# Alvin-Zeng/DRN

Hardware: AMD Instinct MI355X
Metric: clips/sec fwd+bwd (BxT=256x4096 C3D feats) (higher is better)
Workload: dtype bf16; 1 GPU; Charades-STA-shaped C3D features, T=256, D=4096, batch 32/GPU, stage-1 losses; step = fwd+bwd+grad all-reduce+clip(0.5)+Adam; global_batch=32, T=256, D=4096, parallelism=dp1

## Files before the change

drn_amd/csrc/bn.hip:

```cpp
#include "vec.h"
#include "bn_merge.h"
#include "../../include/drn_hip.h"

struct BnFinGroup {
  const float* stats;
  int tiles, M;
  float* scale_shift;
  float* save;
  const float* gamma;
  const float* beta;
  const float* conv_bias;
  float* running_mean;
  float* running_var;
  float momentum, eps;
};
struct BnFinParams {
  int ngroups;
  BnFinGroup g[DRN_MAX_GROUPS];
};

__global__ __launch_bounds__(256 * DRN_MAX_GROUPS) void bn_finalize_kernel(const BnFinParams P, int C) {
  __shared__ double sh[DRN_MAX_GROUPS][16][17];
  __shared__ float s_mean[DRN_MAX_GROUPS][16], s_unb[DRN_MAX_GROUPS][16];
  const int g = threadIdx.x >> 8, t = threadIdx.x & 255;
// ... 388 lines not shown
          const float y = fmaf(u1[k], sc1[k], sh1[k]);
          u1[k] = relu ? fmaxf(y, 0.f) : y;
        }
        if (raw2) {
          float u2[N];
          V16<T>::cvt(ur2[u], u2);
#pragma unroll
          for (int k = 0; k < N; ++k) {
            const float y = fmaf(u2[k], sc2[k], sh2[k]);
            u1[k] += DT<T>::round(relu ? fmaxf(y, 0.f) : y);
          }
        }
#pragma unroll
        for (int k = 0; k < N; ++k) x[k] += DT<T>::round(u1[k]);
      } else if (up) {
        float uu[N];
        V16<T>::cvt(ur[u], uu);
#pragma unroll
        for (int k = 0; k < N; ++k) x[k] += uu[k];
      }
      if (m < row1) {
        V16<T>::store(out + (long)m * ld_out + c0, x);
        if (gated) {
          const float* gp = gate + (long)sq[u] * ldg + c0;
#pragma unroll
          for (int k = 0; k < N; ++k) x[k] *= gp[k];
          V16<T>::store(gated + (long)m * ld_gated + c0, x);
        }
      }
    }
  }
}

extern "C" int drn_bn_train_apply(const DrnBnTrainDesc* d, int n, int C, int relu, int dtype, void* stream) {
  drn_clear_status();
  const char* who = "drn_bn_train_apply";
  DRN_CHECK_ARG(d && n >= 1 && n <= DRN_MAX_GROUPS && C > 0 && C % 64 == 0, "%s: bad args (C must be a multiple of 64)", who);
  DRN_CHECK_ARG(dtype == DRN_F32 || dtype == DRN_BF16, "%s: bad dtype %d", who, dtype);
  const int vn = dtype == DRN_BF16 ? 8 : 4;
  const int RP = 256 / (64 / vn);
  BnTrainParams P;
  memset(&P, 0, sizeof(P));
  P.n = n; P.C = C; P.relu = relu; P.nupd = C / 64;
  long m_all = 0;
  for (int i = 0; i < n; ++i) m_all += d[i].M;
  const long wg4 = ((m_all + 4 * RP - 1) / (4 * RP)) * (C / 64);
  const int rows_wg = 4 * RP * (int)(wg4 > 4096 ? (wg4 + 4095) / 4096 : 1);
  int blocks = P.nupd;
  for (int i = 0; i < n; ++i) {
    const DrnBnTrainDesc& s = d[i];
    DRN_CHECK_ARG(s.raw && s.out && s.stats && s.scale_shift && s.save && s.gamma && s.beta && s.M > 0 && s.L > 0 && s.M % s.L == 0 &&
                  s.tiles == (s.M + 127) / 128, "%s: bad level %d", who, i);
    DRN_CHECK_ARG(!s.up || (s.L % 2 == 0), "%s: upsample-add needs an even sequence length", who);
    DRN_CHECK_ARG((s.gate != nullptr) == (s.gated != nullptr), "%s: gate and gated must come together", who);
    DRN_CHECK_ARG(s.ld_raw % vn == 0 && s.ld_out % vn == 0 && (!s.up || s.ld_up % vn == 0) && (!s.gated || (s.ld_gated % vn == 0 && s.ldg % 4 == 0)),
                  "%s: ld must be 16-byte multiples", who);
    BnTrainLv& G = P.lv[i];
    G.raw = s.raw; G.out = s.out; G.up = s.up; G.gated = s.gated; G.gate = s.gate;
    G.stats = s.stats; G.ss = s.scale_shift; G.save = s.save; G.gamma = s.gamma; G.beta = s.beta; G.conv_bias = s.conv_bias;
    G.running_mean = s.running_mean; G.running_var = s.running_var; G.momentum = s.momentum; G.eps = s.eps;
    G.ld_raw = s.ld_raw; G.ld_out = s.ld_out; G.ld_up = s.ld_up; G.ld_gated = s.ld_gated; G.ldg = s.ldg; G.M = s.M; G.L = s.L;
    G.tiles = s.tiles; G.blk0 = blocks; G.rows_wg = rows_wg;
    blocks += cdiv(s.M, rows_wg) * (C / 64);
    G.chain_next = -1;
    for (int j = 0; j < n && s.up; ++j)
      if (j != i && d[j].out == s.up) {
        DRN_CHECK_ARG(d[j].L * 2 == s.L && d[j].M * 2 == s.M,
                      "%s: level %d adds the output of level %d of the same launch, whose geometry (M=%d L=%d) is not half of its own "
                      "(M=%d L=%d): launch the levels in order", who, i, j, d[j].M, d[j].L, s.M, s.L);
        G.chain_next = j;
        G.up = nullptr;
      }
  }
  for (int i = 0; i < n; ++i) {
    int depth = 1;
    for (int h = P.lv[i].chain_next; h >= 0 && depth <= n; h = P.lv[h].chain_next) ++depth;
    DRN_CHECK_ARG(depth <= 3, "%s: an upsample chain of more than three levels inside one launch (launch the levels in order)", who);
    DRN_CHECK_ARG(P.lv[i].chain_next < 0 || P.lv[i].L % 4 == 0 || P.lv[P.lv[i].chain_next].chain_next < 0,
                  "%s: a three-level chain needs sequence lengths that are multiples of 4", who);
  }
  P.total_blocks = blocks;
  if (dtype == DRN_BF16) bn_train_apply_kernel<bf16_t><<<blocks, 256, 0, (hipStream_t)stream>>>(P);
  else bn_train_apply_kernel<float><<<blocks, 256, 0, (hipStream_t)stream>>>(P);
  return drn_launch_status(who);
}

struct BnBwdLv {
  const void* dout;
  const void* raw;
  void* draw;
  const float* ss;
  const float* save;
  const float* gamma;
  float* dgamma;
  float* dbeta;
  float* partial;
  float* coef;
  int ld_dout, ld_raw, ld_draw, M, accumulate, nblk, yblk0, ablk0;
};
struct BnBwdParams {
  BnBwdLv lv[DRN_MAX_GROUPS];
  int n, C, relu, total_yblk, total_ablk;
};

template <typename T>
__global__ __launch_bounds__(256) void bn_bwd_reduce_kernel(const BnBwdParams P) {
  constexpr int N = V16<T>::N;
  __shared__ float red[2][4][64 * N + 1];
  int li = 0;
#pragma unroll
  for (int i = 1; i < DRN_MAX_GROUPS; ++i)
    if (i < P.n && (int)blockIdx.y >= P.lv[i].yblk0) li = i;
  const BnBwdLv& G = P.lv[li];
  const int C = P.C, relu = P.relu, M = G.M;
// ... 898 lines not shown
```

drn_amd/csrc/bn_merge.h:

```cpp
#pragma once
#include "common.h"

enum { BN_ST_PLAIN = 0, BN_ST_TAGGED = 2 };
struct BnTagged {
  unsigned want;
  int* timeouts;
};
__device__ __forceinline__ unsigned long long bn_tag_pack(float v, unsigned tag) {
  return ((unsigned long long)tag << 32) | (unsigned long long)__float_as_uint(v);
}
__device__ __forceinline__ unsigned long long bn_ld_pair(const unsigned long long* p) {
  return __hip_atomic_load(p, __ATOMIC_RELAXED, __HIP_MEMORY_SCOPE_AGENT);
}
__device__ __forceinline__ bool bn_wait_expired(const long long t0, int* timeouts) {
  __builtin_amdgcn_s_sleep(32);
  if (wall_clock64() - t0 <= 200000000LL) return false;
  __hip_atomic_fetch_add(timeouts, 1, __ATOMIC_RELAXED, __HIP_MEMORY_SCOPE_AGENT);
  return true;
}

__device__ __forceinline__ void bn_wait_slabs(const void* st_, const int slabs, const int C, const int c_first, const BnTagged tg) {
  const unsigned long long* p = (const unsigned long long*)st_ + c_first;
  const int lane = threadIdx.x & 63;
  const long long t0 = wall_clock64();
  for (int s0 = 0; s0 < slabs; s0 += 64) {
    const int s = s0 + lane;
    bool ready = s >= slabs;
    for (;;) {
      if (!ready) ready = (unsigned)(bn_ld_pair(p + ((long)s * 2 + 1) * C) >> 32) == tg.want;
      if (__builtin_amdgcn_ballot_w64(!ready) == 0) break;
      __builtin_amdgcn_s_sleep(12);
      if (wall_clock64() - t0 > 200000000LL) {
        if (!ready) __hip_atomic_fetch_add(tg.timeouts, 1, __ATOMIC_RELAXED, __HIP_MEMORY_SCOPE_AGENT);
        break;
      }
    }
  }
}

template <int CB, int MODE, int TB = 8>
__device__ __forceinline__ void bn_merge_cols(const void* __restrict__ st_, const int tiles, const int Mrows, const int C,
                                              const int cbase, double (*shd)[CB], double& mean_out, double& var_out,
                                              const BnTagged tg = BnTagged{0u, nullptr}) {
#pragma clang fp contract(off)
  constexpr int KMAX = 16;
  const int ci = threadIdx.x % CB, j = threadIdx.x / CB;
  const float* __restrict__ p = (const float*)st_ + cbase;
  const unsigned long long* __restrict__ pt = (const unsigned long long*)st_ + cbase;
  auto at = [&](int k, int which) -> unsigned { return (unsigned)(k * 2 + which) * (unsigned)C + (unsigned)ci; };
  auto ld = [&](int k, int which) -> float {
    if constexpr (MODE == BN_ST_TAGGED) return __uint_as_float((unsigned)bn_ld_pair(pt + at(k, which)));
    else return p[at(k, which)];
  };
  const bool cached = tiles <= 4 * KMAX;
  float c0[KMAX], c1[KMAX];
  double s = 0.0;
  if (cached) {
    if constexpr (MODE == BN_ST_TAGGED) {
      const long long t0 = wall_clock64();
#pragma unroll
      for (int hb = 0; hb < KMAX / TB; ++hb) {
        if (hb > 0 && tiles <= 4 * TB * hb) {
#pragma unroll
          for (int i = hb * TB; i < KMAX; ++i) c0[i] = c1[i] = 0.f;
          break;
        }
        for (;;) {
          bool ok = true;
#pragma unroll
          for (int i = hb * TB; i < (hb + 1) * TB; ++i) {
            const int k = min(j + 4 * i, tiles - 1);
            const unsigned long long v0 = bn_ld_pair(pt + at(k, 0)), v1 = bn_ld_pair(pt + at(k, 1));
            ok &= (unsigned)(v0 >> 32) == tg.want && (unsigned)(v1 >> 32) == tg.want;
            c0[i] = __uint_as_float((unsigned)v0);
            c1[i] = __uint_as_float((unsigned)v1);
          }
          if (ok || bn_wait_expired(t0, tg.timeouts)) break;
        }
      }
// ... 71 lines not shown
```

drn_amd/csrc/gemm_nt.hip:

```cpp
#include "gemm_nt_kernel.h"

bool drn_nt_w4_eligible(const DrnGemmDesc* d, int ngroups, int dtype);
int drn_nt_w4_launch(const GemmParams& P, int total, hipStream_t stream);
bool drn_nt_w4c_eligible(const DrnGemmDesc* d, int ngroups, int dtype);
int drn_nt_w4c_launch(const GemmParams& P, int total, hipStream_t stream, int ksplit, bool eval = false);
bool drn_nt_w4h_eligible(const DrnGemmDesc* d, int ngroups, int dtype, bool* conv_out);
int drn_nt_w4h_launch(const GemmParams& P, int total, bool conv, hipStream_t stream, int ksplit, bool eval = false);

static int nt_kind(const DrnGemmDesc* d, int ngroups, int dtype, int tile, int ksplit, bool planes256) {
  if (tile == 256 && ksplit == 1 && drn_tuning(DRN_TUNE_NT_W4) > 0 && drn_nt_w4_eligible(d, ngroups, dtype)) return DRN_NT_KIND_W4;
  if (tile == 256 && (planes256 || (ksplit == 1 && drn_tuning(DRN_TUNE_NT_W4C) > 0)) && drn_nt_w4c_eligible(d, ngroups, dtype))
    return DRN_NT_KIND_W4C;
  return tile == 256 ? DRN_NT_KIND_TILE256 : DRN_NT_KIND_TILE128;
}

static int launch_nt(const DrnGemmDesc* d, int ngroups, int dtype, hipStream_t stream, int ksplit_arg = 1, float* ws = nullptr,
                     int* counters = nullptr, bool planes256 = false, bool plan_only = false, const DrnBnApplyDesc* ev = nullptr,
                     int ev_relu = 0) {
  const int ksplit = ksplit_arg & 0xffff;
  const int xchg = ksplit_arg & (DRN_XCHG_CONFIRM | DRN_XCHG_NONE);
  DRN_CHECK_ARG(ngroups >= 1 && ngroups <= DRN_MAX_GROUPS, "drn_gemm_nt: ngroups=%d out of range", ngroups);
  DRN_CHECK_ARG(dtype == DRN_F32 || dtype == DRN_BF16, "drn_gemm_nt: bad dtype %d", dtype);
  const int ch = dtype == DRN_BF16 ? 8 : 4;
  long big_tiles = 0;
  bool fast = true;
  for (int g = 0; g < ngroups; ++g) {
    const DrnGemmDesc& s = d[g];
    DRN_CHECK_ARG(s.A && s.B && s.C, "drn_gemm_nt: null operand in group %d", g);
    DRN_CHECK_ARG(s.M > 0 && s.N > 0 && s.Cin > 0 && s.taps >= 1 && s.stride >= 1, "drn_gemm_nt: bad dims in group %d", g);
    DRN_CHECK_ARG(s.Cin % ch == 0 && s.lda % ch == 0 && s.ldb % ch == 0,
                  "drn_gemm_nt: Cin/lda/ldb must be multiples of %d elements (16 bytes); got Cin=%d lda=%d ldb=%d", ch,
                  s.Cin, s.lda, s.ldb);
    DRN_CHECK_ARG(((uintptr_t)s.A & 15) == 0 && ((uintptr_t)s.B & 15) == 0, "drn_gemm_nt: A/B must be 16-byte aligned");
    DRN_CHECK_ARG(s.Lout > 0 && s.Lsrc > 0 && s.M % s.Lout == 0, "drn_gemm_nt: M=%d not a multiple of Lout=%d", s.M, s.Lout);
    big_tiles += (long)cdiv(s.M, 256) * cdiv(s.N, 256);
    if (s.Cin % (8 * ch) != 0 || (s.mode == 1 && s.stride > 2)) fast = false;
  }
  const int big_min = drn_tuning(DRN_TUNE_EXP0) > 0 ? drn_tuning(DRN_TUNE_EXP0) : 200;
  int tile = big_tiles >= big_min ? 256 : 128;
  GemmParams P;
  memset(&P, 0, sizeof(P));
  P.ngroups = ngroups;
  P.ksplit = ksplit | (ksplit > 1 && counters ? (xchg & DRN_XCHG_NONE ? 0 : xchg & DRN_XCHG_CONFIRM ? DRN_XCHG_CONFIRM : DRN_XCHG_READBACK) : 0);
  P.ws = ws;
  P.counters = counters;
  P.xcd_swizzle = 3;
  if (drn_tuning(DRN_TUNE_EXP0 + 3) > 0) P.xcd_swizzle = drn_tuning(DRN_TUNE_EXP0 + 3) - 1;
  if (ksplit > 1) tile = planes256 ? 256 : 128;
  bool w4h = false, w4h_conv = false;
  if (tile == 128 && !planes256 && drn_tuning(DRN_TUNE_NT_W4H) > 0 && drn_nt_w4h_eligible(d, ngroups, dtype, &w4h_conv)) {
    long th = 0;
    int min_ksteps = 1 << 30;
    for (int g = 0; g < ngroups; ++g) {
      th += (long)(d[g].M / 256) * (d[g].N / 128);
      const int ksteps = d[g].taps * d[g].Cin / 64, per = cdiv(ksteps, ksplit);
      min_ksteps = min(min_ksteps, ksteps - (cdiv(ksteps, per) - 1) * per);
      if (cdiv(ksteps, per) != ksplit) min_ksteps = 0;
    }
    w4h = ksplit == 1 ? th >= drn_tuning(DRN_TUNE_NT_W4H)
                      : (ngroups == 1 && th * ksplit >= drn_tuning(DRN_TUNE_NT_W4H) && min_ksteps >= 2 && th <= DRN_QD_COUNTERS && ws && counters);
  }
  const int tile_m = w4h ? 256 : tile, tile_n = w4h ? 128 : tile;
  int total = 0;
  for (int g = 0; g < ngroups; ++g) {
    const DrnGemmDesc& s = d[g];
    GemmProb& p = P.p[g];
    p.A = s.A; p.B = s.B; p.C = s.C; p.C2 = s.C2; p.bias = s.bias; p.gate = s.gate; p.stats = s.stats;
    p.M = s.M; p.N = s.N; p.K = s.taps * s.Cin; p.Cin = s.Cin; p.taps = s.taps; p.stride = s.stride; p.pad = s.pad;
    p.mode = s.mode; p.Lout = s.Lout; p.Lsrc = s.Lsrc; p.lda = s.lda; p.ldb = s.ldb; p.ldc = s.ldc; p.ldg = s.ldg; p.ldc2 = s.ldc2;
    p.accumulate = s.accumulate;
    p.out_f32 = s.out_f32;
    p.sumsq = s.sumsq;
    if (ev) { p.ev_ss = ev[g].scale_shift; p.ev_relu = ev_relu ? 1 : 0; }
    p.gb_act = s.gb_act; p.gb_dct = s.gb_dct; p.gb_dgate = s.gb_dgate; p.gb_dsum = s.gb_dsum; p.gb_ld_act = s.gb_ld_act; p.gb_ldt = s.gb_ldt;
    p.tiles_n = cdiv(s.N, tile_n);
    p.tile_start = total;
    total += cdiv(s.M, tile_m) * p.tiles_n;
  }
  int max_ksteps = 0;
  for (int g = 0; g < ngroups; ++g) max_ksteps = max(max_ksteps, cdiv(cdiv(d[g].taps * d[g].Cin, 8 * ch), ksplit));
  const bool deep8 = tile == 128 &&
                     ((drn_tuning(DRN_TUNE_NT_DEEP) > 0 && (long)total * ksplit <= drn_tuning(DRN_TUNE_NT_DEEP)) ||
                      (drn_tuning(DRN_TUNE_NT_DEEP2) > 0 && (long)total * ksplit <= drn_tuning(DRN_TUNE_NT_DEEP2) &&
                       max_ksteps <= drn_tuning(DRN_TUNE_NT_DEEP_KS)));
  static bool attr_set = false;
  if (!attr_set) {
#define NT_ATTR(TT, SS, ...) \
    (void)hipFuncSetAttribute((const void*)conv_gemm_nt_kernel<TT, SS, true, __VA_ARGS__>, hipFuncAttributeMaxDynamicSharedMemorySize, 163840); \
    (void)hipFuncSetAttribute((const void*)conv_gemm_nt_kernel<TT, SS, false, __VA_ARGS__>, hipFuncAttributeMaxDynamicSharedMemorySize, 163840)
    NT_ATTR(float, 2, 2, 4, 8, 4); NT_ATTR(bf16_t, 2, 2, 4, 8, 4);
    NT_ATTR(float, 2, 2, 4, 4, 2); NT_ATTR(bf16_t, 2, 2, 4, 4, 2);
    NT_ATTR(float, 4, 2, 4, 4, 2); NT_ATTR(bf16_t, 4, 2, 4, 4, 2);
#undef NT_ATTR
#define NT_ATTR(TT, SS, ...) \
    (void)hipFuncSetAttribute((const void*)conv_gemm_nt_eval_kernel<TT, SS, true, __VA_ARGS__>, hipFuncAttributeMaxDynamicSharedMemorySize, 163840); \
    (void)hipFuncSetAttribute((const void*)conv_gemm_nt_eval_kernel<TT, SS, false, __VA_ARGS__>, hipFuncAttributeMaxDynamicSharedMemorySize, 163840)
    NT_ATTR(float, 2, 2, 4, 8, 4); NT_ATTR(bf16_t, 2, 2, 4, 8, 4);
    NT_ATTR(float, 2, 2, 4, 4, 2); NT_ATTR(bf16_t, 2, 2, 4, 4, 2);
    NT_ATTR(float, 4, 2, 4, 4, 2); NT_ATTR(bf16_t, 4, 2, 4, 4, 2);
#undef NT_ATTR
    attr_set = true;
  }
#define NT_LAUNCH(TT, SS, THREADS, LDS, ...) do { \
    P.nblocks = total; \
    if (ev && fast) conv_gemm_nt_eval_kernel<TT, SS, true, __VA_ARGS__><<<dim3(total, ksplit), THREADS, LDS, stream>>>(P); \
    else if (ev) conv_gemm_nt_eval_kernel<TT, SS, false, __VA_ARGS__><<<dim3(total, ksplit), THREADS, LDS, stream>>>(P); \
    else if (fast) conv_gemm_nt_kernel<TT, SS, true, __VA_ARGS__><<<dim3(total, ksplit), THREADS, LDS, stream>>>(P); \
    else conv_gemm_nt_kernel<TT, SS, false, __VA_ARGS__><<<dim3(total, ksplit), THREADS, LDS, stream>>>(P); } while (0)
  const int kind = w4h ? DRN_NT_KIND_W4H : nt_kind(d, ngroups, dtype, tile, ksplit, planes256);
  if (ev && kind == DRN_NT_KIND_W4) {
    drn_set_error("drn_conv_bn_eval: gemm_nt_w4_kernel (large plain products) has no BatchNorm epilogue");
    return DRN_ERR_UNSUPPORTED;
  }
  if (plan_only) return kind;
  if (kind == DRN_NT_KIND_W4H) {
    P.nblocks = total;
    return drn_nt_w4h_launch(P, total, w4h_conv, stream, ksplit, ev != nullptr);
  }
  for (int g = 0; g < ngroups; ++g)
    DRN_CHECK_ARG(!d[g].sumsq || (kind == DRN_NT_KIND_W4 && d[g].out_f32 && !d[g].bias && !d[g].accumulate && ngroups == 1),
                  "drn_gemm_nt: DrnGemmDesc::sumsq needs a single fp32-output launch on gemm_nt_w4_kernel without bias / accumulate "
                  "(ask drn_gemm_nt_plan first)");
  for (int g = 0; g < ngroups; ++g) {
    const DrnGemmDesc& s = d[g];
    if (!s.gb_act) continue;
    DRN_CHECK_ARG(kind == DRN_NT_KIND_W4C && ngroups == 1 && ksplit == 1 && s.mode == 1 && s.gate && s.gb_dct && s.gb_dgate && s.gb_dsum &&
                      !s.bias && !s.C2 && !s.stats && !s.accumulate && (s.Lout == 32 || s.Lout == 64 || s.Lout == 128 || s.Lout == 256) &&
                      s.gb_ld_act % 8 == 0 && s.gb_ldt % 8 == 0 && !((uintptr_t)s.gb_act & 15) && !((uintptr_t)s.gb_dct & 15) && s.ldg >= s.N,
                  "drn_gemm_nt: DrnGemmDesc::gb_* needs a single bf16 data-gradient launch on gemm_nt_w4c_kernel (ask drn_gemm_nt_plan "
                  "first) with gate and all three outputs set, clips of 32 / 64 / 128 / 256 rows, no bias / C2 / stats / accumulate");
  }
  if (kind == DRN_NT_KIND_W4) {
    P.nblocks = total;
    return drn_nt_w4_launch(P, total, stream);
  }
  if (kind == DRN_NT_KIND_W4C) {
    P.nblocks = total;
    return drn_nt_w4c_launch(P, total, stream, ksplit, ev != nullptr);
  }
  if (planes256) {
    drn_set_error("drn_gemm_nt_splitk256: the problem is not one gemm_nt_w4c_kernel runs (bf16, k = 3 / stride 1 / pad 1, M and N multiples of 256, Cin of 64)");
    return DRN_ERR_UNSUPPORTED;
// ... 207 lines not shown
```

drn_amd/csrc/gemm_nt_kernel.h:

```cpp
#pragma once
#include <type_traits>
#include "common.h"
#include "bn_merge.h"
#include "../../include/drn_hip.h"



struct GemmProb {
  const void* A;
  const void* B;
  void* C;
  void* C2;
  union {
    const float* bias;
    const float* ev_ss;
  };
  const float* gate;
  float* stats;
  int M, N, K;
  int Cin, taps, stride, pad, mode;
  int Lout, Lsrc;
  int lda, ldb, ldc, ldg, ldc2;
  union {
    int accumulate;
// ... 395 lines not shown
      const int mrow0 = m0 + wr * (MI * 16) + ch * 32;
#pragma unroll
      for (int mi2 = 0; mi2 < 2; ++mi2)
#pragma unroll
        for (int r = 0; r < 4; ++r)
#pragma unroll
          for (int ni = 0; ni < NI; ++ni)
            *((float*)(wbuf + (mi2 * 16 + (l >> 4) * 4 + r) * PITCHF) + ni * 16 + (l & 15)) = acc[ch * 2 + mi2][ni][r];
      wave_lds_sync();
#pragma unroll
      for (int it = 0; it < 32 / RPIF; ++it) {
        const int rl = it * RPIF + l / LPRF, cv = l % LPRF;
        const int m = mrow0 + rl, n = n0 + wc * (NI * 16) + cv * 4;
        if (m < M && n < N) {
          f32x4 v = *(const f32x4*)(wbuf + rl * PITCHF + cv * 16);
          float* g = Cf + ((long)m * pr.ldc + n);
          if (pr.bias)
#pragma unroll
            for (int k = 0; k < 4; ++k) v[k] += n + k < N ? pr.bias[n + k] : 0.f;
          if (vec4 && n + 4 <= N && !pr.accumulate) {
            *(f32x4*)g = v;
          } else {
#pragma unroll
            for (int k = 0; k < 4; ++k)
              if (n + k < N) g[k] = pr.accumulate ? g[k] + v[k] : v[k];
          }
        }
      }
      wave_lds_sync();
    }
    return;
  }
  auto bn_stats = [&](float* shs) { nt_bn_stats<WM, WN, MI, NI, BN_ST_PLAIN>(acc, shs, pr.stats, M, N, m0, n0, tm); };

  T* __restrict__ Cg = (T*)pr.C;
  T* __restrict__ C2g = (T*)pr.C2;
  constexpr int VEC = 16 / (int)sizeof(T);
  const bool vec_ok = (pr.ldc % VEC == 0) && (((uintptr_t)Cg & 15) == 0) &&
                      (!C2g || ((pr.ldc2 % VEC == 0) && (((uintptr_t)C2g & 15) == 0)));
  const bool stats_first = !vec_ok;
  if (!EVAL && stats_first && pr.stats) {
    bn_stats((float*)smem);
    __syncthreads();
  }
  if (vec_ok) {
    constexpr int WCOLS = NI * 16;
    constexpr int PITCH = WCOLS * (int)sizeof(T) + 16;
    constexpr int LPR = WCOLS * (int)sizeof(T) / 16;
    constexpr int RPI = 64 / LPR;
    char* wbuf = smem + w * (32 * PITCH);
    float bias_v[NI], scale_v[NI];
#pragma unroll
    for (int ni = 0; ni < NI; ++ni) {
      const int n = n0 + wc * (NI * 16) + ni * 16 + (l & 15);
      if constexpr (EVAL) {
        scale_v[ni] = n < N ? pr.ev_ss[n] : 0.f;
        bias_v[ni] = n < N ? pr.ev_ss[N + n] : 0.f;
      } else {
        bias_v[ni] = (pr.bias && n < N) ? pr.bias[n] : 0.f;
      }
    }
    (void)scale_v;
    const int npass = C2g ? 2 : 1;
#pragma unroll
    for (int ch = 0; ch < MI / 2; ++ch) {
      const int mrow0 = m0 + wr * (MI * 16) + ch * 32;
// ... 743 lines not shown
```

drn_amd/functional.py:

```python
import contextlib
import weakref

import torch

from . import ops
from ._lib import DrnError

class WeightCopies(object):

    _live = []

    def __init__(self):
        self.pack, self.pstack, self.stack, self.shape_stack = {}, {}, {}, {}
        self.epoch = 0
        self.gen = 0
        WeightCopies._live.append(weakref.ref(self))

    def bump_gen(self):
        self.gen += 1

    def bump_epoch(self):
        self.epoch += 1

    def adopt(self, module):
# ... 668 lines not shown
        keep = (draws, xs)
        dWj = _alias(dW)
        _defer(lambda: (keep, ops.gemm_wgrad(wdescs, dWj, Cout, Cin, taps=k, stride=meta.stride, pad=pad, w_layout=1, dtype=code)), dWj)
        dxs = [None] * nl
        if any(ctx.needs_input_grad[7 + l] for l in range(nl)):
            wd = packed(ctx.weight_obj, (1, 2, 0), code)
            tail = meta.tail if (meta.tail is not None and nl == 1 and k in (1, 3) and meta.tail.usable(Cin, Cout, dt)) else None
            ncols = Cin - tail.P if tail is not None else Cin
            descs = []
            for l in range(nl):
                B, L, Lo, M, ld = geo[l]
                dx = torch.empty((B, L, Cin), dtype=dt, device=dev)
                descs.append(ops.gemm_desc(draws[l], wd, dx, B * L, ncols, Cout, taps=k, stride=meta.stride, pad=pad, mode=1,
                                           Lout=L, Lsrc=Lo, ldc=Cin))
                dxs[l] = dx
            gctx = tail.gate_ctx if tail is not None else None
            if (gctx is not None and k == 3 and meta.stride == 1 and gctx[2:] == (geo[0][0], geo[0][1], ncols)
                    and ops.gemm_nt_plan(descs, code) == ops.NT_KIND_W4C):
                Z, gate0, B, T, D = gctx
                dZT = torch.empty((D, B * T), dtype=dt, device=dev)
                dgate0 = torch.empty((B, D), dtype=torch.float32, device=dev)
                dsum0 = torch.empty((B, D), dtype=torch.float32, device=dev)
                descs = [ops.gemm_desc(draws[0], wd, dxs[0], B * T, ncols, Cout, taps=k, stride=1, pad=pad, mode=1, Lout=T, Lsrc=T, ldc=Cin,
                                       gate=gate0, ldg=gate0.stride(0),
                                       gate_bwd=dict(act=Z, ld_act=D, dct=dZT, ldt=B * T, dgate=dgate0, dsum=dsum0))]
                tail.gate_out = (dZT, dgate0, dsum0)
            ops.gemm_nt(descs, code)
            if tail is not None:
                B, L, Lo, M, ld = geo[0]
                tail.backward(draws[0], wd, B, L, Lo, Cout, Cin, k, meta.stride, pad, code)
        return (None, dW, None, dgamma, dbeta, dgate, dup) + tuple(dxs)


def conv_block(xs, conv, bn, training, dtype, gate=None, up=None, relu=True, tail=None):
    meta = ConvMeta(conv.stride[0], bn, training, dtype, relu, tail=tail)
    res = _ConvBlockFn.apply(meta, conv.weight, conv.bias, bn.weight, bn.bias, gate, up, *xs)
    if gate is not None:
        return list(res[:-1]), res[-1]
    return list(res), None


def conv0_mx8_weights(weight, gate0, D, Dp, out=None):
    Cout, P = int(weight.shape[0]), int(weight.shape[1]) - int(D)
    S, dev = int(gate0.shape[0]), weight.device
    w = packed(weight, (2, 0, 1), ops.F32)
    if out is None:
        out = (torch.empty((S, 3, Cout, Dp), dtype=torch.uint8, device=dev), torch.empty((S, 3, Cout, Dp // 32), dtype=torch.uint8, device=dev),
               torch.empty((3, Cout, P), dtype=torch.bfloat16, device=dev) if P else None)
    wcodes, wscales, wpos = out
    ops.gate_quantize_weights_mx8(w[:, :, :D], gate0, D, Dp, wcodes, wscales)
    if P:
        wpos.copy_(w[:, :, D:])
    return wcodes, wscales, wpos


def conv0_mx8_block(index, wq, pair_q, pair_v, vids, L, conv, bn, gate, dt):
    wcodes, wscales, wpos = wq
    Q, Cout, dev, code = int(pair_q.numel()), int(conv.weight.shape[0]), index.codes.device, code_of(dt)
    raw = torch.empty((Q, L, Cout), dtype=dt, device=dev)
    ops.conv0_mx8(index.codes, index.scales, index.pos if index.P else None, index.pad_row, index.prop_off, wcodes, wscales, wpos, pair_q,
                  pair_v, vids, raw, L, index.Dp, index.P)
    ss = torch.empty((2, Cout), dtype=torch.float32, device=dev)
    ops.bn_eval_scale_shift(Cout, bn.weight, bn.bias, conv.bias, bn.running_mean, bn.running_var, bn.eps, ss)
    out = torch.empty((Q, L, Cout), dtype=dt, device=dev)
    gated = torch.empty((Q, L, Cout), dtype=dt, device=dev) if gate is not None else None
    ops.bn_apply_multi([dict(raw=raw, ld_raw=Cout, ss=ss, out=out, ld_out=Cout, M=Q * L, L=L, up=None, ld_up=0, gate=gate, gated=gated,
                             ld_gated=Cout)], Cout, code, relu=True)
# ... 863 lines not shown
```

drn_amd/model/fcos.py:

```python
import math
import types

import torch
from torch import nn

from .. import functional as DF
from .inference import make_fcos_postprocessor
from .loss import make_fcos_loss_evaluator


class Scale(nn.Module):

    def __init__(self, init_value=1.0):
        super(Scale, self).__init__()
        self.scale = nn.Parameter(torch.FloatTensor([init_value]))

    def forward(self, input):
        return input * self.scale


class LevelList(list):
    flat = None


class FCOSHead(torch.nn.Module):
    compute_dtype = torch.float32

    def __init__(self, cfg, in_channels):
        super(FCOSHead, self).__init__()
        num_classes = cfg["fcos_num_class"] - 1
        cls_tower, bbox_tower = [], []
        for _ in range(cfg["fcos_conv_layers"]):
            cls_tower += [nn.Conv1d(in_channels, in_channels, 3, stride=1, padding=1), nn.BatchNorm1d(in_channels), nn.ReLU()]
            bbox_tower += [nn.Conv1d(in_channels, in_channels, 3, stride=1, padding=1), nn.BatchNorm1d(in_channels), nn.ReLU()]
        self.add_module('cls_tower', nn.Sequential(*cls_tower))
        self.add_module('bbox_tower', nn.Sequential(*bbox_tower))
        self.cls_logits = nn.Conv1d(in_channels, num_classes, kernel_size=3, stride=1, padding=1)
        self.bbox_pred = nn.Conv1d(in_channels, 2, kernel_size=3, stride=1, padding=1)
        self.centerness = nn.Conv1d(in_channels, 1, kernel_size=3, stride=1, padding=1)
# ... 27 lines not shown
            for i in range(nlayers):
                ct, _ = DF.conv_block(ct, self.cls_tower[3 * i], self.cls_tower[3 * i + 1], self.training, dt)
                bt, _ = DF.conv_block(bt, self.bbox_tower[3 * i], self.bbox_tower[3 * i + 1], self.training, dt)
            return [torch.cat([c, b], dim=2) for c, b in zip(ct, bt)]
        cc, cb, bc, bb = self.cls_tower[0], self.cls_tower[1], self.bbox_tower[0], self.bbox_tower[1]
        conv = types.SimpleNamespace(weight=DF.stack_params([cc.weight, bc.weight]), bias=DF.stack_params([cc.bias, bc.bias]),
                                     stride=(1,))
        track = cb.running_mean is not None
        rm, rv = self._stacked_running(cb, bb) if track else (None, None)
        bn = types.SimpleNamespace(weight=DF.stack_params([cb.weight, bb.weight]), bias=DF.stack_params([cb.bias, bb.bias]),
                                   running_mean=rm, running_var=rv, num_batches_tracked=None, momentum=cb.momentum,
                                   eps=cb.eps, track_running_stats=cb.track_running_stats)
        out, _ = DF.conv_block(xs, conv, bn, self.training, dt)
        if self.training and track:
            DF.bump_bn_counter(cb.num_batches_tracked, len(xs)); DF.bump_bn_counter(bb.num_batches_tracked, len(xs))
        return out

    def _stacked_running(self, cb, bb):
        C = cb.num_features
        st = getattr(self, "_tower_stats", None)
        if st is not None:
            rm, rv = st
            if cb.running_mean.data_ptr() == rm.data_ptr() and bb.running_mean.data_ptr() == rm[C:].data_ptr() and \
                    cb.running_var.data_ptr() == rv.data_ptr() and bb.running_var.data_ptr() == rv[C:].data_ptr():
                return rm, rv
        with torch.no_grad():
            rm = torch.cat([cb.running_mean, bb.running_mean])
            rv = torch.cat([cb.running_var, bb.running_var])
            cb.running_mean, bb.running_mean = rm[:C], rm[C:]
            cb.running_var, bb.running_var = rv[:C], rv[C:]
        self._tower_stats = (rm, rv)
        return rm, rv

    def forward_nlc(self, xs):
        dt = self.compute_dtype
        C = xs[0].shape[2]
        ctbt = self._towers(xs)
        scales = DF.stack_params([s.scale for s in self.scales[:len(xs)]])
        K = self.cls_logits.weight.shape[0]
        if K <= 2:
            logits, reg = DF.head_out(ctbt, [(self.cls_logits, None), (self.bbox_pred, scales)], cols=[0, C], dtype=dt)
        else:
            W, b = self.cls_logits.weight, self.cls_logits.bias
            part = lambda c0: types.SimpleNamespace(weight=W[c0:c0 + 2], bias=b[c0:c0 + 2])
            l0, reg = DF.head_out(ctbt, [(part(0), None), (self.bbox_pred, scales)], cols=[0, C], dtype=dt)
            rest = [DF.head_out(ctbt, [(part(c0), None)], cols=[0], dtype=dt)[0] for c0 in range(2, K, 2)]
            logits = torch.cat([l0] + rest, dim=1)
        mix, _ = DF.conv_block(ctbt, self.mix_fc[0], self.mix_fc[1], self.training, dt)
        iouf, _ = DF.conv_block(mix, self.iou_scores[0], self.iou_scores[1], self.training, dt)
        (iou,) = DF.head_out(iouf, [(self.iou_scores[3], None)], cols=[0], dtype=dt)
        return logits, reg, iou, [(x.shape[0], x.shape[1]) for x in xs]

    @staticmethod
    def split_levels(flat, geo):
        out, r = LevelList(), 0
        for B, L in geo:
            out.append(flat[r:r + B * L].view(B, L, -1).permute(0, 2, 1))
            r += B * L
        out.flat = flat
        return out

    def forward(self, x):
        logits, reg, iou, geo = self.forward_nlc([DF.as_nlc(f, self.compute_dtype) for f in x])
        DF.flush_bn_counters()
        return self.split_levels(logits, geo), self.split_levels(reg, geo), [], self.split_levels(iou, geo)


class FCOSModule(torch.nn.Module):

    def __init__(self, cfg, in_channels):
        super(FCOSModule, self).__init__()
        self.head = FCOSHead(cfg, in_channels)
        self.is_first_stage = cfg['is_first_stage']
        self.box_selector_test = make_fcos_postprocessor(cfg)
        self.loss_evaluator = make_fcos_loss_evaluator(cfg)
        self.fpn_strides = cfg["fpn_stride"]
        self.loss_evaluator.fpn_strides = list(self.fpn_strides)
        self.box_selector_test.strides = [float(s) for s in self.fpn_strides]
        self._locations = {}

    def forward(self, features, targets=None):
        box_cls, box_regression, centerness, iou_scores = self.head(features)
        locations = self.compute_locations(features)
        if self.training:
            return self._forward_train(locations, box_cls, box_regression, targets, iou_scores)
        return self._forward_test(locations, box_cls, box_regression, targets, iou_scores)

    def _forward_train(self, locations, box_cls, box_regression, targets, iou_scores):
        loss_box_cls, loss_box_reg, loss_iou = self.loss_evaluator(
            locations, box_cls, box_regression, targets, iou_scores, self.is_first_stage)
        return None, self._loss_dict(loss_box_cls, loss_box_reg, loss_iou)

    def _forward_test(self, locations, box_cls, box_regression, targets, iou_scores):
        boxes = self.box_selector_test(locations, box_cls, box_regression, iou_scores)
        loss_box_cls, loss_box_reg, loss_iou = self.loss_evaluator(
            locations, box_cls, box_regression, targets, iou_scores, self.is_first_stage)
        return boxes, self._loss_dict(loss_box_cls, loss_box_reg, loss_iou)

    def _loss_dict(self, loss_box_cls, loss_box_reg, loss_iou):
        d = DF.LossDict(loss_cls=loss_box_cls, loss_reg=loss_box_reg, loss_iou=loss_iou)
        d.total = getattr(self.loss_evaluator, "last_total", None)
        return d

    def compute_locations(self, features):
        return [self.compute_locations_per_level(f.size(-1), self.fpn_strides[l], f.device) for l, f in enumerate(features)]

    def compute_locations_per_level(self, t, stride, device):
        key = (int(t), stride, str(device))
        loc = self._locations.get(key)
        if loc is None:
            shifts_t = torch.arange(0, t * stride, step=stride, dtype=torch.float32, device=device)
            loc = self._locations[key] = shifts_t.reshape(-1) + stride / 2
        return loc


# ... 3 lines not shown
```

drn_amd/model/main_model.py:

```python
import types

import torch
import torch.nn.functional as F
import torch.nn as nn

from .. import functional as DF
from .. import ops
from .._lib import DrnError
from .backbone import Backbone
from .basic_blocks import conv_with_kaiming_uniform
from .fcos import FCOSHead, build_fcos
from .FPN import FPN
from .language_module import QueryEncoder


class mainModel(nn.Module):
    def __init__(self, vocab_size, dataset_configs, hidden_dim=512, embed_dim=300, bidirection=True,
                 graph_node_features=1024, compute_dtype=torch.float32):
        super(mainModel, self).__init__()
        dataset_configs = vars(dataset_configs) if not isinstance(dataset_configs, dict) else dataset_configs
        self.first_output_dim = dataset_configs["first_output_dim"]
        self.fpn_feature_dim = dataset_configs["fpn_feature_dim"]
        self.feature_dim = dataset_configs[dataset_configs['feature_type']]['feature_dim']
        self.query_encoder = QueryEncoder(vocab_size, hidden_dim, embed_dim, dataset_configs["lstm_layers"], bidirection)
# ... 73 lines not shown
            raise DrnError("drn_amd.mainModel runs on an MI355X only (inputs on %s); no CPU fallback" % props_features.device)
        dt = self.compute_dtype
        want_wgrad = self.prop_fc.weight.requires_grad and torch.is_grad_enabled()
        pad = self._front_pad(props_features.shape[2])
        if pad:
            props_features = F.pad(props_features, (0, pad))
            fc = types.SimpleNamespace(weight=F.pad(self.prop_fc.weight, (0, pad, 0, pad)), bias=F.pad(self.prop_fc.bias, (0, pad)))
        else:
            fc = self.prop_fc
        prep = DF.input_prep(props_features, props_start_end, fc, dt, want_wgrad,
                             split_gate=getattr(self, "split_gate", False) if split_gate is None else split_gate,
                             position_transform=self.position_transform)
        prep.fc = fc
        return prep

    def _front_pad(self, D):
        return (-D) % 64 if (self.compute_dtype == torch.bfloat16 and D % 8) else 0

    def forward_front(self, query_tokens, query_length, props_features, props_start_end, gates=None, prep=None):
        if prep is None:
            prep = self.prepare_input(props_features, props_start_end)
        if gates is None:
            gates = self.encode_query(query_tokens, query_length)
        pad = self._front_pad(self.feature_dim)
        gate0 = F.pad(gates[0], (0, pad)) if pad else gates[0]
        g0, tail = DF.input_stage(prep, prep.fc, gate0, self.position_transform, with_tail=True)
        g0._drn_tail = tail
        return g0, gates

    def _trunk_heads(self, g0, gates, conv0=None):
        backbone_feats = self.backbone_net.forward_from_stage(g0, gates, tail=getattr(g0, "_drn_tail", None), conv0=conv0)
        feats = self.fpn.forward_nlc(backbone_feats)
        head = self.fcos.head
        logits, reg, iou, geo = head.forward_nlc(feats)
        box_cls, box_reg, iou_scores = (FCOSHead.split_levels(t, geo) for t in (logits, reg, iou))
        if self.taps is not None:
            for i, f in enumerate(backbone_feats):
                self.taps["backbone_net.forward_conv%d" % i] = f.permute(0, 2, 1)
            for i, f in enumerate(feats):
                self.taps["fpn.fpn_layer%d" % (i + 1)] = f.permute(0, 2, 1)
            self.taps["head"] = (box_cls, box_reg, [], iou_scores)
        fc = self.fcos
        locations = [fc.compute_locations_per_level(L, fc.fpn_strides[l], logits.device) for l, (_, L) in enumerate(geo)]
        return locations, box_cls, box_reg, iou_scores

    def forward_trunk(self, g0, gates, gt_start_end):
        locations, box_cls, box_reg, iou_scores = self._trunk_heads(g0, gates)
        fc = self.fcos
        targets = gt_start_end if gt_start_end.dtype in (torch.float32, torch.float64) else gt_start_end.float()
        if self.training:
            res = fc._forward_train(locations, box_cls, box_reg, targets, iou_scores)
        else:
            res = fc._forward_test(locations, box_cls, box_reg, targets, iou_scores)
        DF.flush_bn_counters()
        return res

    def forward_heads_shared(self, query_tokens, query_length, props_features, props_start_end, video_index=None, query_index=None,
                             gates=None):
        if self.training:
            raise DrnError("forward_heads_shared is inference only: call model.eval() first")
        if torch.is_grad_enabled():
            raise DrnError("forward_heads_shared is inference only: run it under torch.no_grad()")
        for t in (props_features, props_start_end) + ((query_tokens,) if gates is None else tuple(gates)):
            if not t.is_cuda:
                raise DrnError("drn_amd.mainModel runs on an MI355X only (inputs on %s); no CPU fallback" % t.device)
        V, T, _ = props_features.shape
        dev = props_features.device
# ... 96 lines not shown
```

drn_amd/ops.py:

```python
import ctypes

import torch

from . import _lib
from ._lib import GemmDesc, WgradDesc, check, lib

F32, BF16 = 0, 1


def dtype_code(t):
    if t.dtype == torch.float32:
        return F32
    if t.dtype == torch.bfloat16:
        return BF16
    raise _lib.DrnError("unsupported dtype %s (float32 / bfloat16 only)" % t.dtype)


def _p(t):
    return ctypes.c_void_p(t.data_ptr()) if t is not None else None


def _stream():
    return ctypes.c_void_p(torch.cuda.current_stream().cuda_stream)

# ... 81 lines not shown
        check(kind, "drn_gemm_nt_plan")
    return kind


KSPLIT_W4H = True


def _ksplit_w4h(descs, dtype):
    if not KSPLIT_W4H or dtype != BF16 or len(descs) != 1:
        return 1
    d = descs[0]
    if d.M % 256 or d.N % 128 or d.Cin % 64:
        return 1
    tiles, nkt = (d.M // 256) * (d.N // 128), (d.taps * d.Cin) // 64
    if tiles > 128 or nkt < 96:
        return 1
    ks = min(8, KSPLIT_WGS // tiles, nkt // 24)
    while ks > 1 and -(-nkt // -(-nkt // ks)) != ks:
        ks -= 1
    if ks < 2:
        return 1
    arr = (GemmDesc * 1)(d)
    return ks if lib().drn_gemm_nt_splitk_plan(arr, 1, ks, dtype) == NT_KIND_W4H else 1


KSPLIT_CONFIRM_ATOMIC, KSPLIT_CONFIRM_NONE = 0x20000, 0x80000
XCHG_CONFIRM = "2"


def _ksplit_arg(ks):
    return ks | (KSPLIT_CONFIRM_NONE if XCHG_CONFIRM == "0" else KSPLIT_CONFIRM_ATOMIC if XCHG_CONFIRM == "1" else 0)


def gemm_nt(descs, dtype):
    arr = (GemmDesc * len(descs))(*descs)
    flops = sum(2.0 * d.M * d.N * d.taps * d.Cin for d in descs)
    ks = _ksplit_w4h(descs, dtype)
    if ks > 1:
        d0 = descs[0]
        dev = torch.device("cuda", torch.cuda.current_device())
        ws = torch.empty(ks * d0.M * d0.N, dtype=torch.float32, device=dev)
        tag = "gemm_nt[bf16] g=1 M=%d N=%d K=%d mode=%d splitK=%d(w4h)" % (d0.M, d0.N, d0.taps * d0.Cin, d0.mode, ks)
        return _timed(tag, flops, lambda: check(lib().drn_gemm_nt_splitk_grouped(arr, 1, _ksplit_arg(ks), _p(ws), _p(_counters(dev)), dtype, _stream()),
                                                "drn_gemm_nt_splitk_grouped"))
    ks = _ksplit256(descs, dtype)
    if ks > 1:
        d0 = descs[0]
        dev = torch.device("cuda", torch.cuda.current_device())
        ws = workspace(ks * d0.M * d0.N, dev)
        tag = "gemm_nt[bf16] g=1 M=%d N=%d K=%d mode=%d splitK256=%d" % (d0.M, d0.N, d0.taps * d0.Cin, d0.mode, ks)
        return _timed(tag, flops, lambda: check(lib().drn_gemm_nt_splitk256(arr, ks, _p(ws), dtype, _stream()), "drn_gemm_nt_splitk256"))
    ks = _ksplit(descs, dtype)
    if ks > 1:
        d0 = descs[0]
        dev = torch.device("cuda", torch.cuda.current_device())
        tiles = sum(((d.M + 127) // 128) * ((d.N + 127) // 128) for d in descs)
        ws = torch.empty(ks * tiles * 128 * 128, dtype=torch.float32, device=dev)
        tag = "gemm_nt[%s] g=%d M=%d N=%d K=%d mode=%d splitK=%d" % ("bf16" if dtype == BF16 else "f32", len(descs),
                                                                     sum(d.M for d in descs), d0.N, d0.taps * d0.Cin, d0.mode, ks)
        return _timed(tag, flops, lambda: check(lib().drn_gemm_nt_splitk_grouped(arr, len(descs), _ksplit_arg(ks), _p(ws), _p(_counters(dev)),
                                                                                 dtype, _stream()), "drn_gemm_nt_splitk_grouped"))
    d0 = descs[0]
    tag = "gemm_nt[%s] g=%d M=%d N=%d K=%d mode=%d" % ("bf16" if dtype == BF16 else "f32", len(descs),
                                                      sum(d.M for d in descs), d0.N, d0.taps * d0.Cin, d0.mode)
    _timed(tag, flops, lambda: check(lib().drn_gemm_nt(arr, len(descs), dtype, _stream()), "drn_gemm_nt"))


# ... 1069 lines not shown
```

Measured before the change: 16780 clips/s.

## Skip IoU branch output in stage-1 training, keep only BN statistics

In first-stage training the IoU scores are unused by the losses, so the iou_scores conv block now runs in statistics-only mode. The GEMM computes BatchNorm partial stats without storing its output, and a new small kernel finalizes scale/shift and updates the running statistics without the apply pass. The head_out projection and its backward are skipped entirely. This keeps BN running-stat side effects identical while removing the output write, the normalize/ReLU pass and the IoU head's forward and backward work.

```diff
diff --git a/drn_amd/csrc/bn.hip b/drn_amd/csrc/bn.hip
--- a/drn_amd/csrc/bn.hip
+++ b/drn_amd/csrc/bn.hip
@@ -444,6 +444,37 @@
   }
 }
 
+__global__ __launch_bounds__(256 * DRN_MAX_GROUPS) void bn_train_stats_kernel(const BnTrainParams P) {
+  __shared__ double shd[DRN_MAX_GROUPS][4][64];
+  __shared__ double s_mean[DRN_MAX_GROUPS][64], s_var[DRN_MAX_GROUPS][64];
+  const int C = P.C, g = threadIdx.x >> 8, t = threadIdx.x & 255;
+  const int cbase = blockIdx.x * 64;
+  {
+    const BnTrainLv& G = P.lv[g];
+    double mean, var;
+    bn_merge_cols<64, BN_ST_PLAIN>(G.stats, G.tiles, G.M, C, cbase, shd[g], mean, var, BnTagged{0u, nullptr}, t);
+    if (t < 64) {
+      s_mean[g][t] = mean;
+      s_var[g][t] = var;
+    }
+  }
+  __syncthreads();
+  if (threadIdx.x < 64) {
+    const int c = cbase + threadIdx.x;
+    for (int k = 0; k < P.n; ++k) {
+      const BnTrainLv& G = P.lv[k];
+      const double mean = s_mean[k][threadIdx.x], var = s_var[k][threadIdx.x];
+      float sc, sh, invstd;
+      bn_scale_shift(mean, var, G.eps, G.gamma[c], G.beta[c], sc, sh, invstd);
+      G.ss[c] = sc;
+      G.ss[C + c] = sh;
+      G.save[c] = (float)mean;
+      G.save[C + c] = invstd;
+      bn_running_update(mean, var, G.M, G.momentum, G.conv_bias ? G.conv_bias[c] : 0.f, G.running_mean, G.running_var, c);
+    }
+  }
+}
+
 extern "C" int drn_bn_train_apply(const DrnBnTrainDesc* d, int n, int C, int relu, int dtype, void* stream) {
   drn_clear_status();
   const char* who = "drn_bn_train_apply";
@@ -459,9 +490,12 @@
   const long wg4 = ((m_all + 4 * RP - 1) / (4 * RP)) * (C / 64);
   const int rows_wg = 4 * RP * (int)(wg4 > 4096 ? (wg4 + 4095) / 4096 : 1);
   int blocks = P.nupd;
+  const bool stats_only = !d[0].out;
   for (int i = 0; i < n; ++i) {
     const DrnBnTrainDesc& s = d[i];
-    DRN_CHECK_ARG(s.raw && s.out && s.stats && s.scale_shift && s.save && s.gamma && s.beta && s.M > 0 && s.L > 0 && s.M % s.L == 0 &&
+    DRN_CHECK_ARG(!s.out == stats_only, "%s: out is NULL (statistics only) in some levels and not in others", who);
+    DRN_CHECK_ARG(!stats_only || (!s.up && !s.gate && !s.gated), "%s: level %d has no out (statistics only): up / gate / gated do not apply", who, i);
+    DRN_CHECK_ARG((stats_only || (s.raw && s.out)) && s.stats && s.scale_shift && s.save && s.gamma && s.beta && s.M > 0 && s.L > 0 && s.M % s.L == 0 &&
                   s.tiles == (s.M + 127) / 128, "%s: bad level %d", who, i);
     DRN_CHECK_ARG(!s.up || (s.L % 2 == 0), "%s: upsample-add needs an even sequence length", who);
     DRN_CHECK_ARG((s.gate != nullptr) == (s.gated != nullptr), "%s: gate and gated must come together", who);
@@ -492,6 +526,10 @@
                   "%s: a three-level chain needs sequence lengths that are multiples of 4", who);
   }
   P.total_blocks = blocks;
+  if (stats_only) {
+    bn_train_stats_kernel<<<P.nupd, 256 * n, 0, (hipStream_t)stream>>>(P);
+    return drn_launch_status(who);
+  }
   if (dtype == DRN_BF16) bn_train_apply_kernel<bf16_t><<<blocks, 256, 0, (hipStream_t)stream>>>(P);
   else bn_train_apply_kernel<float><<<blocks, 256, 0, (hipStream_t)stream>>>(P);
   return drn_launch_status(who);
diff --git a/drn_amd/csrc/bn_merge.h b/drn_amd/csrc/bn_merge.h
--- a/drn_amd/csrc/bn_merge.h
+++ b/drn_amd/csrc/bn_merge.h
@@ -41,10 +41,10 @@
 template <int CB, int MODE, int TB = 8>
 __device__ __forceinline__ void bn_merge_cols(const void* __restrict__ st_, const int tiles, const int Mrows, const int C,
                                               const int cbase, double (*shd)[CB], double& mean_out, double& var_out,
-                                              const BnTagged tg = BnTagged{0u, nullptr}) {
+                                              const BnTagged tg = BnTagged{0u, nullptr}, const int tid = threadIdx.x) {
 #pragma clang fp contract(off)
   constexpr int KMAX = 16;
-  const int ci = threadIdx.x % CB, j = threadIdx.x / CB;
+  const int ci = tid % CB, j = tid / CB;
   const float* __restrict__ p = (const float*)st_ + cbase;
   const unsigned long long* __restrict__ pt = (const unsigned long long*)st_ + cbase;
   auto at = [&](int k, int which) -> unsigned { return (unsigned)(k * 2 + which) * (unsigned)C + (unsigned)ci; };
diff --git a/drn_amd/csrc/gemm_nt.hip b/drn_amd/csrc/gemm_nt.hip
--- a/drn_amd/csrc/gemm_nt.hip
+++ b/drn_amd/csrc/gemm_nt.hip
@@ -24,9 +24,15 @@
   const int ch = dtype == DRN_BF16 ? 8 : 4;
   long big_tiles = 0;
   bool fast = true;
+  bool stats_only = false;
   for (int g = 0; g < ngroups; ++g) {
     const DrnGemmDesc& s = d[g];
-    DRN_CHECK_ARG(s.A && s.B && s.C, "drn_gemm_nt: null operand in group %d", g);
+    DRN_CHECK_ARG(s.A && s.B && (s.C || s.stats), "drn_gemm_nt: null operand in group %d", g);
+    if (!s.C) {
+      DRN_CHECK_ARG(!s.C2 && !s.gate && !s.accumulate && !s.out_f32 && !s.sumsq && !s.gb_act && !ev && !planes256,
+                    "drn_gemm_nt: group %d has no C (statistics only): C2 / gate / accumulate / out_f32 / sumsq / gb_* do not apply", g);
+      stats_only = true;
+    }
     DRN_CHECK_ARG(s.M > 0 && s.N > 0 && s.Cin > 0 && s.taps >= 1 && s.stride >= 1, "drn_gemm_nt: bad dims in group %d", g);
     DRN_CHECK_ARG(s.Cin % ch == 0 && s.lda % ch == 0 && s.ldb % ch == 0,
                   "drn_gemm_nt: Cin/lda/ldb must be multiples of %d elements (16 bytes); got Cin=%d lda=%d ldb=%d", ch,
@@ -48,7 +54,7 @@
   if (drn_tuning(DRN_TUNE_EXP0 + 3) > 0) P.xcd_swizzle = drn_tuning(DRN_TUNE_EXP0 + 3) - 1;
   if (ksplit > 1) tile = planes256 ? 256 : 128;
   bool w4h = false, w4h_conv = false;
-  if (tile == 128 && !planes256 && drn_tuning(DRN_TUNE_NT_W4H) > 0 && drn_nt_w4h_eligible(d, ngroups, dtype, &w4h_conv)) {
+  if (tile == 128 && !planes256 && !stats_only && drn_tuning(DRN_TUNE_NT_W4H) > 0 && drn_nt_w4h_eligible(d, ngroups, dtype, &w4h_conv)) {
     long th = 0;
     int min_ksteps = 1 << 30;
     for (int g = 0; g < ngroups; ++g) {
@@ -107,7 +113,9 @@
     else if (ev) conv_gemm_nt_eval_kernel<TT, SS, false, __VA_ARGS__><<<dim3(total, ksplit), THREADS, LDS, stream>>>(P); \
     else if (fast) conv_gemm_nt_kernel<TT, SS, true, __VA_ARGS__><<<dim3(total, ksplit), THREADS, LDS, stream>>>(P); \
     else conv_gemm_nt_kernel<TT, SS, false, __VA_ARGS__><<<dim3(total, ksplit), THREADS, LDS, stream>>>(P); } while (0)
-  const int kind = w4h ? DRN_NT_KIND_W4H : nt_kind(d, ngroups, dtype, tile, ksplit, planes256);
+  const int kind = w4h ? DRN_NT_KIND_W4H
+                       : stats_only ? (tile == 256 ? DRN_NT_KIND_TILE256 : DRN_NT_KIND_TILE128)
+                                    : nt_kind(d, ngroups, dtype, tile, ksplit, planes256);
   if (ev && kind == DRN_NT_KIND_W4) {
     drn_set_error("drn_conv_bn_eval: gemm_nt_w4_kernel (large plain products) has no BatchNorm epilogue");
     return DRN_ERR_UNSUPPORTED;
diff --git a/drn_amd/csrc/gemm_nt_kernel.h b/drn_amd/csrc/gemm_nt_kernel.h
--- a/drn_amd/csrc/gemm_nt_kernel.h
+++ b/drn_amd/csrc/gemm_nt_kernel.h
@@ -451,6 +451,10 @@
     return;
   }
   auto bn_stats = [&](float* shs) { nt_bn_stats<WM, WN, MI, NI, BN_ST_PLAIN>(acc, shs, pr.stats, M, N, m0, n0, tm); };
+  if (!EVAL && !pr.C) {
+    bn_stats((float*)smem);
+    return;
+  }
 
   T* __restrict__ Cg = (T*)pr.C;
   T* __restrict__ C2g = (T*)pr.C2;
diff --git a/drn_amd/functional.py b/drn_amd/functional.py
--- a/drn_amd/functional.py
+++ b/drn_amd/functional.py
@@ -724,7 +724,45 @@
         return (None, dW, None, dgamma, dbeta, dgate, dup) + tuple(dxs)
 
 
-def conv_block(xs, conv, bn, training, dtype, gate=None, up=None, relu=True, tail=None):
+def _conv_block_stats(xs, conv, bn, dtype):
+    code = code_of(dtype)
+    weight, cbias, gamma, beta = conv.weight.detach(), conv.bias, bn.weight.detach(), bn.bias.detach()
+    Cout, Cin, k = weight.shape
+    if Cout % 64:
+        raise DrnError("conv_block(stats_only=True) needs a multiple of 64 output channels (drn_bn_train_apply), got %d" % Cout)
+    if bn.momentum is None:
+        raise DrnError("cumulative-average BatchNorm (momentum=None) is not supported")
+    pad, stride = (k - 1) // 2, conv.stride[0]
+    wp = packed(conv.weight, (0, 2, 1), code)
+    dev = weight.device
+    track = bn.track_running_stats and bn.running_mean is not None
+    descs, levels = [], []
+    for x in xs:
+        if x.dtype != dtype:
+            raise DrnError("activation dtype %s != compute dtype %s" % (x.dtype, dtype))
+        B, L, C, ld = geom(x)
+        assert C == Cin, (C, Cin)
+        Lo = (L + 2 * pad - k) // stride + 1
+        M = B * Lo
+        st = torch.empty(((M + 127) // 128, 2, Cout), dtype=torch.float32, device=dev)
+        descs.append(ops.gemm_desc(x.detach(), wp, None, M, Cout, Cin, taps=k, stride=stride, pad=pad, Lout=Lo, Lsrc=L, lda=ld, stats=st))
+        levels.append(dict(raw=None, ld_raw=0, out=None, ld_out=0, M=M, L=Lo, stats=st, tiles=(M + 127) // 128,
+                           ss=torch.empty((2, Cout), dtype=torch.float32, device=dev),
+                           save=torch.empty((2, Cout), dtype=torch.float32, device=dev), gamma=gamma, beta=beta,
+                           conv_bias=cbias.detach() if cbias is not None else None,
+                           running_mean=bn.running_mean if track else None, running_var=bn.running_var if track else None,
+                           momentum=bn.momentum, eps=bn.eps))
+    ops.gemm_nt_stats(descs, code)
+    ops.bn_train_apply(levels, Cout, code, relu=True)
+    if track and bn.num_batches_tracked is not None:
+        bump_bn_counter(bn.num_batches_tracked, len(xs))
+
+
+def conv_block(xs, conv, bn, training, dtype, gate=None, up=None, relu=True, tail=None, stats_only=False):
+    if stats_only:
+        if not training or gate is not None or up is not None:
+            raise DrnError("conv_block(stats_only=True) is the train-mode block without gate / up")
+        return _conv_block_stats(xs, conv, bn, dtype)
     meta = ConvMeta(conv.stride[0], bn, training, dtype, relu, tail=tail)
     res = _ConvBlockFn.apply(meta, conv.weight, conv.bias, bn.weight, bn.bias, gate, up, *xs)
     if gate is not None:
diff --git a/drn_amd/model/fcos.py b/drn_amd/model/fcos.py
--- a/drn_amd/model/fcos.py
+++ b/drn_amd/model/fcos.py
@@ -5,6 +5,7 @@
 from torch import nn
 
 from .. import functional as DF
+from .. import ops
 from .inference import make_fcos_postprocessor
 from .loss import make_fcos_loss_evaluator
 
@@ -98,7 +99,7 @@
         self._tower_stats = (rm, rv)
         return rm, rv
 
-    def forward_nlc(self, xs):
+    def forward_nlc(self, xs, need_iou=True):
         dt = self.compute_dtype
         C = xs[0].shape[2]
         ctbt = self._towers(xs)
@@ -113,12 +114,19 @@
             rest = [DF.head_out(ctbt, [(part(c0), None)], cols=[0], dtype=dt)[0] for c0 in range(2, K, 2)]
             logits = torch.cat([l0] + rest, dim=1)
         mix, _ = DF.conv_block(ctbt, self.mix_fc[0], self.mix_fc[1], self.training, dt)
-        iouf, _ = DF.conv_block(mix, self.iou_scores[0], self.iou_scores[1], self.training, dt)
-        (iou,) = DF.head_out(iouf, [(self.iou_scores[3], None)], cols=[0], dtype=dt)
+        if need_iou:
+            iouf, _ = DF.conv_block(mix, self.iou_scores[0], self.iou_scores[1], self.training, dt)
+            (iou,) = DF.head_out(iouf, [(self.iou_scores[3], None)], cols=[0], dtype=dt)
+        else:
+            DF.conv_block(mix, self.iou_scores[0], self.iou_scores[1], self.training, dt, stats_only=True)
+            DF.packed(self.iou_scores[3].weight, (0, 2, 1), ops.F32)
+            iou = None
         return logits, reg, iou, [(x.shape[0], x.shape[1]) for x in xs]
 
     @staticmethod
     def split_levels(flat, geo):
+        if flat is None:
+            return None
         out, r = LevelList(), 0
         for B, L in geo:
             out.append(flat[r:r + B * L].view(B, L, -1).permute(0, 2, 1))
@@ -126,8 +134,8 @@
         out.flat = flat
         return out
 
-    def forward(self, x):
-        logits, reg, iou, geo = self.forward_nlc([DF.as_nlc(f, self.compute_dtype) for f in x])
+    def forward(self, x, need_iou=True):
+        logits, reg, iou, geo = self.forward_nlc([DF.as_nlc(f, self.compute_dtype) for f in x], need_iou=need_iou)
         DF.flush_bn_counters()
         return self.split_levels(logits, geo), self.split_levels(reg, geo), [], self.split_levels(iou, geo)
 
@@ -144,9 +152,11 @@
         self.loss_evaluator.fpn_strides = list(self.fpn_strides)
         self.box_selector_test.strides = [float(s) for s in self.fpn_strides]
         self._locations = {}
+        self.taps = None
 
     def forward(self, features, targets=None):
-        box_cls, box_regression, centerness, iou_scores = self.head(features)
+        need_iou = not (self.training and self.is_first_stage and self.taps is None)
+        box_cls, box_regression, centerness, iou_scores = self.head(features, need_iou=need_iou)
         locations = self.compute_locations(features)
         if self.training:
             return self._forward_train(locations, box_cls, box_regression, targets, iou_scores)
diff --git a/drn_amd/model/main_model.py b/drn_amd/model/main_model.py
--- a/drn_amd/model/main_model.py
+++ b/drn_amd/model/main_model.py
@@ -129,7 +129,8 @@
         backbone_feats = self.backbone_net.forward_from_stage(g0, gates, tail=getattr(g0, "_drn_tail", None), conv0=conv0)
         feats = self.fpn.forward_nlc(backbone_feats)
         head = self.fcos.head
-        logits, reg, iou, geo = head.forward_nlc(feats)
+        need_iou = not (self.training and self.fcos.is_first_stage and self.taps is None)
+        logits, reg, iou, geo = head.forward_nlc(feats, need_iou=need_iou)
         box_cls, box_reg, iou_scores = (FCOSHead.split_levels(t, geo) for t in (logits, reg, iou))
         if self.taps is not None:
             for i, f in enumerate(backbone_feats):
diff --git a/drn_amd/ops.py b/drn_amd/ops.py
--- a/drn_amd/ops.py
+++ b/drn_amd/ops.py
@@ -137,7 +137,22 @@
     return ks | (KSPLIT_CONFIRM_NONE if XCHG_CONFIRM == "0" else KSPLIT_CONFIRM_ATOMIC if XCHG_CONFIRM == "1" else 0)
 
 
+def gemm_nt_stats(descs, dtype):
+    global kernel_timer
+    if any(d.C for d in descs):
+        raise _lib.DrnError("gemm_nt_stats: every descriptor must come without C")
+    saved, kernel_timer = kernel_timer, None
+    try:
+        _gemm_nt(descs, dtype)
+    finally:
+        kernel_timer = saved
+
+
 def gemm_nt(descs, dtype):
+    _gemm_nt(descs, dtype)
+
+
+def _gemm_nt(descs, dtype):
     arr = (GemmDesc * len(descs))(*descs)
     flops = sum(2.0 * d.M * d.N * d.taps * d.Cin for d in descs)
     ks = _ksplit_w4h(descs, dtype)
```

New measurement: 16920 clips/s (median of 6 runs). No clear change (+0.8%).
